# Daaohame/RAHT-3DGS-codec

Measured on AMD Instinct MI355X. Metric: M-Gaussians/s fwd+inv RAHT, 59-ch SH3 3DGS, higher is better.
Workload: dtype f32 (xyz columns: f64); 1 GPU; cfg3: 2999072 Gaussians (3000000 draws/GPU, J=12, 59 channels), fwd RAHT + quantize/reorder + dequantize/un-reorder + inv RAHT (quantization fused into the transform kernels); the 3 xyz columns carried in float64 inside the same launches (raht_fwd_quant_mixed / raht_dequant_inv_mixed): the reference's integers on every column; rows_per_gpu=2999072, channels=59, depth_J=12, engine=tile, quantize=True, parallelism=1 GPU, world=1

## Files before the change

### raht-3dgs-codec_amd/csrc/schedule.hip

```cpp
#include "raht_common.h"

#include <algorithm>
#include <atomic>

namespace raht {

__global__ void compact_scatter_kernel(const uint32_t *in, const uint32_t *flag, const uint32_t *pos, uint32_t *out, int64_t n);

__global__ void stage_survivor_kernel(const uint32_t *__restrict__ rows, int64_t n, int R, int64_t N,
                                      const int32_t *__restrict__ wl, const int32_t *__restrict__ wr,
                                      const uint8_t *__restrict__ lvl, int top_level,
                                      uint32_t *__restrict__ survivor)
{
    const int64_t j = (int64_t)blockIdx.x * blockDim.x + threadIdx.x;
    if (j >= n) return;
    const int64_t r = rows ? rows[j] : j;
    const int64_t t = j / R;
    const int64_t j0 = t * R, j1 = j0 + R;
    const int64_t start = rows ? rows[j0] : j0;
    const int64_t end = (j1 < n) ? (rows ? (int64_t)rows[j1] : j1) : N;
    const bool merged = (r > 0) && ((int)lvl[r] < top_level) && (r - wl[r] >= start) && (r + wr[r] <= end);
    survivor[j] = merged ? 0u : 1u;
}

// ... 378 lines not shown
        P.prog = st.prog;
        const size_t lds = st.rows ? (size_t)R * 4 : 0;
        const unsigned grid = (unsigned)st.n_tiles;
        by_lane_slots(R, [&](auto spl) {
            hipLaunchKernelGGL(tile_program_kernel<decltype(spl)::value>, dim3(grid), dim3(64), lds, s, P, plan->N, plan->top_level, plan->wsum);
        });
        RAHT_HIP_CHECK(hipGetLastError());
        st.prog_stride = P.stride; st.prog_ab = P.ab; st.prog_compact = P.compact != 0;
        built = true;
    }
    if (built) {
        if (!sc->ready) RAHT_HIP_CHECK(hipEventCreateWithFlags(&sc->ready.ev, hipEventDisableTiming));
        RAHT_HIP_CHECK(hipEventRecord(sc->ready, s));
        sc->ready_on = s;
    }
    return RAHT_OK;
}

__global__ void top_resolve_kernel(const uint32_t *__restrict__ rows, int64_t n, const int32_t *__restrict__ wl,
                                   const int32_t *__restrict__ wr, const uint8_t *__restrict__ lvl,
                                   const int64_t *__restrict__ wsum, int top_level, uint32_t *__restrict__ pj,
                                   double *__restrict__ ab, uint8_t *__restrict__ bucket, uint32_t *__restrict__ is_root)
{
    const int64_t e = (int64_t)blockIdx.x * blockDim.x + threadIdx.x;
    if (e >= n) return;
    const int64_t r = rows ? (int64_t)rows[e] : e;
    const int l = (int)lvl[r];
    const bool merged = (r > 0) && (l < top_level);
    is_root[e] = merged ? 0u : 1u;
    bucket[e] = merged ? (uint8_t)l : (uint8_t)63;
    uint32_t rec = 0;
    double a = 0.0, b = 0.0;
    if (merged) {
        const int64_t want = r - wl[r];
        int64_t p = want;
        if (rows) {
            int64_t lo = 0, hi = e - 1;
            while (lo < hi) {
                const int64_t mid = (lo + hi) >> 1;
                if ((int64_t)rows[mid] < want) lo = mid + 1; else hi = mid;
            }
            p = lo;
        }
        double w0, w1;
        pair_weights(r, wl[r], wr[r], wsum, w0, w1);
        const double den = w0 + w1;
        a = sqrt(w0 / den);
        b = sqrt(w1 / den);
        rec = (uint32_t)p | ((uint32_t)e << 16);
    }
    pj[e] = rec; ab[2 * e] = a; ab[2 * e + 1] = b;
}

__global__ void top_gather_kernel(const uint32_t *__restrict__ perm, uint32_t n_merges, const uint32_t *__restrict__ pj,
                                  const double *__restrict__ ab, uint32_t *__restrict__ t_pj,
                                  float *__restrict__ t_ab32, double *__restrict__ t_ab64)
{
    const uint32_t k = blockIdx.x * blockDim.x + threadIdx.x;
    if (k >= n_merges) return;
    const uint32_t e = perm[k];
    t_pj[k] = pj[e];
    const double a = ab[2 * e], b = ab[2 * e + 1];
    t_ab64[2 * k] = a; t_ab64[2 * k + 1] = b;
    t_ab32[2 * k] = (float)a; t_ab32[2 * k + 1] = (float)b;
}

__global__ void top_root_rank_kernel(const uint32_t *__restrict__ is_root, const uint32_t *__restrict__ pos, int64_t n,
                                     uint32_t *__restrict__ t_root)
{
    const int64_t e = (int64_t)blockIdx.x * blockDim.x + threadIdx.x;
    if (e < n) t_root[e] = is_root[e] ? pos[e] : 0xffffffffu;
}

static hipError_t gather_stage_meta(const raht_plan *plan, Stage &st, hipStream_t s)
{
    const size_t n = (size_t)st.n_entries;
    hipError_t e = hipSuccess;
    if ((e = st.e_wl.alloc(n)) != hipSuccess || (e = st.e_wr.alloc(n)) != hipSuccess || (e = st.e_lvl.alloc(n)) != hipSuccess ||
        (e = st.e_pos.alloc(n)) != hipSuccess) return e;
    hipLaunchKernelGGL(gather_meta_kernel, dim3((unsigned)ceil_div((int64_t)n, 256)), dim3(256), 0, s, st.rows, (int64_t)n, plan->wl,
                       plan->wr, plan->lvl, plan->inv_order, st.e_wl, st.e_wr, st.e_lvl, st.e_pos);
    return hipSuccess;
}

static int build_top_stage(raht_plan *plan, int64_t n, hipStream_t s, Stage &st)
{
    st.is_top = true;
    st.n_entries = n;
    st.n_tiles = 1;
    st.tile_rows = (int)n;
    const uint32_t *rows = st.rows;
    const unsigned gb = (unsigned)ceil_div(n, 256);
    if (rows) RAHT_HIP_CHECK(gather_stage_meta(plan, st, s));
    Scratch buf(sizeof(double) * 2 * (size_t)n + sizeof(uint32_t) * (4 * (size_t)n + 66) + (size_t)n, s);
    if (!buf.ok()) return RAHT_ERR_NOMEM;
    double *ab = buf.as<double>();
    uint32_t *pj = (uint32_t *)(ab + 2 * n), *is_root = pj + n, *pos = is_root + n, *perm = pos + n, *boff = perm + n,
             *total = boff + 65;
    uint8_t *bucket = (uint8_t *)(total + 1);
    hipLaunchKernelGGL(top_resolve_kernel, dim3(gb), dim3(256), 0, s, rows, n, plan->wl, plan->wr, plan->lvl, plan->wsum,
                       plan->top_level, pj, ab, bucket, is_root);
    RAHT_RET(exclusive_scan_u32(is_root, pos, n, total, s));
    RAHT_HIP_CHECK(st.t_root.alloc((size_t)n));
    hipLaunchKernelGGL(top_root_rank_kernel, dim3(gb), dim3(256), 0, s, is_root, pos, n, st.t_root);
    RAHT_RET(bucket_sort_u8(bucket, perm, n, 6, boff, s));
    RAHT_RET(read_back_u32(st.t_loff, boff, 65, nullptr, nullptr, 0, s));
    st.n_merges = st.t_loff[63];
    {
        uint32_t *lev = st.t_lev_host;
        int nlev = 0;
        for (int l = 0; l < 63; ++l)
            if (st.t_loff[l + 1] > st.t_loff[l]) { lev[2 * nlev] = st.t_loff[l]; lev[2 * nlev + 1] = st.t_loff[l + 1]; ++nlev; }
        int nbig = nlev;
        while (nbig > 0 && lev[2 * (nbig - 1) + 1] - lev[2 * (nbig - 1)] <= 64) --nbig;
        const size_t lds_budget = 160 * 1024 - 1024;
        while (nbig < nlev && (size_t)n * 16 + (size_t)(st.n_merges - lev[2 * nbig]) * 20 > lds_budget) ++nbig;
        st.t_nlev = nlev; st.t_nbig = nbig;
        st.t_small_start = (nbig < nlev) ? lev[2 * nbig] : st.n_merges;
        RAHT_HIP_CHECK(st.t_lev.alloc(2 * 64));
        RAHT_HIP_CHECK(hipMemcpyAsync(st.t_lev, lev, sizeof(uint32_t) * 2 * (size_t)std::max(nlev, 1), hipMemcpyHostToDevice, s));
    }
    const size_t nm = std::max<size_t>(st.n_merges, 1);
    RAHT_HIP_CHECK(st.t_pj.alloc(nm));
    RAHT_HIP_CHECK(st.t_ab32.alloc(2 * nm));
    RAHT_HIP_CHECK(st.t_ab64.alloc(2 * nm));
    if (st.n_merges)
        hipLaunchKernelGGL(top_gather_kernel, dim3((unsigned)ceil_div(st.n_merges, 256)), dim3(256), 0, s, perm, st.n_merges,
                           pj, ab, st.t_pj, st.t_ab32, st.t_ab64);
    return RAHT_OK;
}

constexpr int SB_THREADS = 256, SB_ITEMS = 8, SB_BLOCK = SB_THREADS * SB_ITEMS;
constexpr int SCHED_SPEC_MAX = 8;
enum { SK_NONE = 0, SK_TILE = 1, SK_TOP = 2 };

struct SchedState {
    uint32_t n[SCHED_SPEC_MAX + 2];
    uint32_t kind[SCHED_SPEC_MAX + 2];
    uint32_t finished;
    uint32_t last_stage, last_is_top;
    uint32_t trouble;
    uint32_t top[4];
};
constexpr int SCHED_STATE_WORDS = sizeof(SchedState) / 4;

__device__ __forceinline__ uint32_t block_sum_256(uint32_t v, uint32_t *red )
{
#pragma unroll
    for (int d = 32; d >= 1; d >>= 1) v += __shfl_xor(v, d, 64);
    if ((threadIdx.x & 63) == 0) red[threadIdx.x >> 6] = v;
    __syncthreads();
    const uint32_t t = red[0] + red[1] + red[2] + red[3];
    __syncthreads();
    return t;
}

__device__ __forceinline__ void sched_state_init(SchedState *S, uint32_t n0, uint32_t kind0)
// ... 104 lines not shown
#pragma unroll
        for (int q = 0; q < SB_ITEMS; ++q) { f[q] = (base + q < n) ? flags[base + q] : 0; mine += f[q]; }
    }
    uint32_t inc = mine;
    const int lane = threadIdx.x & 63, wid = threadIdx.x >> 6;
#pragma unroll
    for (int d = 1; d < 64; d <<= 1) { const uint32_t t = __shfl_up(inc, d, 64); if (lane >= d) inc += t; }
    if (lane == 63) wsum[wid] = inc;
    __syncthreads();
    uint32_t before = 0, block_tot = 0;
#pragma unroll
    for (int w = 0; w < 4; ++w) { if (w < wid) before += wsum[w]; block_tot += wsum[w]; }
    uint32_t pos = block_base + before + inc - mine;
    uint32_t tile = (uint32_t)base / (uint32_t)R;
    uint32_t next_start = tile * (uint32_t)R;
    if (next_start < (uint32_t)base) { ++tile; next_start += (uint32_t)R; }
    uint32_t g_r[SB_ITEMS], g_pos[SB_ITEMS], g_inv[SB_ITEMS];
    int32_t g_wl[SB_ITEMS], g_wr[SB_ITEMS];
    uint8_t g_lv[SB_ITEMS];
    bool keep[SB_ITEMS];
#pragma unroll
    for (int q = 0; q < SB_ITEMS; ++q) {
        const int64_t j = base + q;
        keep[q] = false; g_pos[q] = 0; g_r[q] = (uint32_t)j;
        if (j < n) {
            if ((uint32_t)j == next_start) { surv_off[tile] = pos; ++tile; next_start += (uint32_t)R; }
            if (f[q]) {
                keep[q] = pos < cap_next;
                g_pos[q] = pos;
                if (keep[q] && rows) g_r[q] = rows[j];
                ++pos;
            }
        }
    }
#pragma unroll
    for (int q = 0; q < SB_ITEMS; ++q) {
        g_wl[q] = 0; g_wr[q] = 0; g_lv[q] = 0; g_inv[q] = 0;
        if (keep[q]) { const uint32_t r = g_r[q]; g_wl[q] = p_wl[r]; g_wr[q] = p_wr[r]; g_lv[q] = p_lvl[r]; g_inv[q] = p_inv[r]; }
    }
#pragma unroll
    for (int q = 0; q < SB_ITEMS; ++q)
        if (keep[q]) { const uint32_t o = g_pos[q]; n_rows[o] = g_r[q]; n_wl[o] = g_wl[q]; n_wr[o] = g_wr[q]; n_lvl[o] = g_lv[q]; n_pos[o] = g_inv[q]; }
    if ((int64_t)blockIdx.x == nblk - 1 && threadIdx.x == 0) {
        const uint32_t total = block_base + block_tot;
        surv_off[(n + R - 1) / R] = total;
        S->n[k + 1] = total;
        if (total > cap_next) S->trouble = 1;
        else if (total == n_roots) { S->finished = 1; S->last_stage = (uint32_t)k; S->last_is_top = 0; }
        else if (total >= (uint32_t)n) S->trouble = 2;
        else S->kind[k + 1] = (total <= Rf) ? SK_TOP : SK_TILE;
    }
}

constexpr int ST_THREADS = 1024;
struct SchedTopOut { uint32_t *t_pj; float *t_ab32; double *t_ab64; uint32_t *t_root; uint32_t *t_lev; };

__device__ __forceinline__ void sched_top_body(SchedState *__restrict__ S, int k, int n, const uint32_t *__restrict__ rows,
                                               const int32_t *__restrict__ p_wl, const int32_t *__restrict__ p_wr,
                                               const uint8_t *__restrict__ p_lvl, const int64_t *__restrict__ wsum,
                                               int top_level, const SchedTopOut &O)
{
    __shared__ uint32_t s_rows[RAHT_TOP_MAX_ROWS];
    __shared__ uint32_t hist[64], cursor[64], wtot[ST_THREADS / 64];
    __shared__ uint32_t root_base;
    uint32_t *__restrict__ t_pj = O.t_pj, *__restrict__ t_root = O.t_root, *__restrict__ t_lev = O.t_lev;
    float *__restrict__ t_ab32 = O.t_ab32;
    double *__restrict__ t_ab64 = O.t_ab64;
    const int tid = threadIdx.x, lane = tid & 63, wid = tid >> 6;
    if (tid < 64) hist[tid] = 0;
    if (tid == 0) root_base = 0;
    for (int e = tid; e < n; e += ST_THREADS) s_rows[e] = rows ? rows[e] : (uint32_t)e;
    __syncthreads();
    PL_STAMP(2, 0, 8);
    for (int e0 = 0; e0 < n; e0 += ST_THREADS) {
        const int e = e0 + tid;
        bool root = false;
        if (e < n) {
            const uint32_t r = s_rows[e];
            const int l = (int)p_lvl[r];
            const bool merged = (r > 0) && (l < top_level);
            root = !merged;
            if (merged) atomicAdd(&hist[l], 1u);
        }
        const uint64_t bal = __ballot(root);
        if (lane == 0) wtot[wid] = (uint32_t)__popcll(bal);
        __syncthreads();
        uint32_t before = root_base;
        for (int w = 0; w < wid; ++w) before += wtot[w];
        if (e < n) t_root[e] = root ? before + (uint32_t)__popcll(bal & (((uint64_t)1 << lane) - 1)) : 0xffffffffu;
        __syncthreads();
        if (tid == 0) { uint32_t t = 0; for (int w = 0; w < ST_THREADS / 64; ++w) t += wtot[w]; root_base += t; }
        __syncthreads();
    }
    PL_STAMP(2, 0, 9);
    if (wid == 0) {
        const uint32_t h = (lane < 63) ? hist[lane] : 0u;
        uint32_t inc = h;
#pragma unroll
        for (int d = 1; d < 64; d <<= 1) { const uint32_t t = __shfl_up(inc, d, 64); if (lane >= d) inc += t; }
        const uint32_t first = inc - h;
        cursor[lane] = first;
        const uint32_t n_merges = (uint32_t)__shfl((int)inc, 63, 64);
        const uint64_t nonempty = __ballot(h > 0), below = ((uint64_t)1 << lane) - 1;
        const int nlev = __popcll(nonempty);
        const int my = __popcll(nonempty & below);
        if (h > 0) { t_lev[2 * my] = first; t_lev[2 * my + 1] = first + h; }
        const uint64_t big = __ballot(h > 64);
        int nbig = big ? __popcll(nonempty & (((uint64_t)2 << (63 - __clzll((long long)big))) - 1)) : 0;
        const size_t lds_budget = 160 * 1024 - 1024;
        uint32_t small_start = n_merges;
        for (;;) {
            uint32_t cand = n_merges;
            if (nbig < nlev) {
                const uint64_t owner = __ballot(h > 0 && my == nbig);
                cand = (uint32_t)__shfl((int)first, __ffsll((unsigned long long)owner) - 1, 64);
            }
            if (nbig < nlev && (size_t)n * 16 + (size_t)(n_merges - cand) * 20 > lds_budget) { ++nbig; continue; }
            small_start = cand;
            break;
        }
        if (lane == 0) {
            S->top[0] = n_merges; S->top[1] = (uint32_t)nlev; S->top[2] = (uint32_t)nbig; S->top[3] = small_start;
            S->finished = 1; S->last_stage = (uint32_t)k; S->last_is_top = 1;
        }
    }
    __syncthreads();
    PL_STAMP(2, 0, 10);
    for (int e = tid; e < n; e += ST_THREADS) {
        const uint32_t r = s_rows[e];
        const int l = (int)p_lvl[r];
        if (!((r > 0) && (l < top_level))) continue;
        const int32_t wlr = p_wl[r], wrr = p_wr[r];
        const uint32_t want = r - (uint32_t)wlr;
        int lo = 0, hi = e - 1;
        while (lo < hi) {
            const int mid = (lo + hi) >> 1;
            if (s_rows[mid] < want) lo = mid + 1; else hi = mid;
        }
        double w0, w1;
        pair_weights((int64_t)r, wlr, wrr, wsum, w0, w1);
        const double den = w0 + w1;
        const double a = sqrt(w0 / den), b = sqrt(w1 / den);
        const uint32_t pos = atomicAdd(&cursor[l], 1u);
        t_pj[pos] = (uint32_t)lo | ((uint32_t)e << 16);
        t_ab64[2 * pos] = a; t_ab64[2 * pos + 1] = b;
        t_ab32[2 * pos] = (float)a; t_ab32[2 * pos + 1] = (float)b;
    }
    PL_STAMP(2, 0, 11);
}

struct SchedStageBufs {
    uint32_t *rows[SCHED_SPEC_MAX + 2]; int32_t *wl[SCHED_SPEC_MAX + 2], *wr[SCHED_SPEC_MAX + 2];
    uint8_t *lvl[SCHED_SPEC_MAX + 2]; uint32_t *pos[SCHED_SPEC_MAX + 2], *surv[SCHED_SPEC_MAX + 2];
    uint32_t cap[SCHED_SPEC_MAX + 2];
};

__global__ __launch_bounds__(ST_THREADS) void sched_tail_kernel(SchedState *S, int k_multi, int k_last, SchedStageBufs B, int R, uint32_t Rf,
                                                                uint32_t n_roots, int64_t N, int top_level, uint32_t tail_max,
                                                                const int32_t *__restrict__ p_wl, const int32_t *__restrict__ p_wr,
                                                                const uint8_t *__restrict__ p_lvl, const uint32_t *__restrict__ p_inv,
                                                                const int64_t *__restrict__ wsum, SchedTopOut O, int64_t n_first)
{
    __shared__ uint32_t wcnt[8 * (ST_THREADS / 64)], woff[8 * (ST_THREADS / 64) + 1];
    __shared__ uint32_t s_kind[SCHED_SPEC_MAX + 2], s_n[SCHED_SPEC_MAX + 2];
    const int tid = threadIdx.x, lane = tid & 63, wid = tid >> 6;
    PL_SLOT_DECL;
    PL_STAMP_NEXT();
    if (n_first >= 0) { sched_state_init(S, (uint32_t)n_first, SK_TOP); __builtin_amdgcn_fence(__ATOMIC_RELEASE, "workgroup"); __syncthreads(); }
    if (tid < SCHED_SPEC_MAX + 2) {
        s_kind[tid] = (n_first >= 0) ? (tid == 0 ? (uint32_t)SK_TOP : (uint32_t)SK_NONE) : __atomic_load_n(&S->kind[tid], __ATOMIC_RELAXED);
        s_n[tid] = (n_first >= 0) ? (tid == 0 ? (uint32_t)n_first : 0u) : __atomic_load_n(&S->n[tid], __ATOMIC_RELAXED);
    }
    __syncthreads();
    for (int k = (k_multi == 0) ? 0 : 1; k <= k_last; ++k) {
        const uint32_t kind = s_kind[k], n = s_n[k];
        PL_STAMP_NEXT();
        if (kind == SK_TOP) {
            sched_top_body(S, k, (int)n, B.rows[k], p_wl, p_wr, p_lvl, wsum, top_level, O);
            return;
        }
        if (kind == SK_TILE && k < k_multi) continue;
        if (kind != SK_TILE || n > tail_max || n > B.cap[k] || k == k_last) return;
        const uint32_t *__restrict__ rows = B.rows[k];
        const int32_t *__restrict__ wl = B.wl[k], *__restrict__ wr = B.wr[k];
        const uint8_t *__restrict__ lvl = B.lvl[k];
        uint32_t *__restrict__ surv_off = B.surv[k];
        uint32_t *__restrict__ n_rows = B.rows[k + 1], *__restrict__ n_pos = B.pos[k + 1];
        int32_t *__restrict__ n_wl = B.wl[k + 1], *__restrict__ n_wr = B.wr[k + 1];
        uint8_t *__restrict__ n_lvl = B.lvl[k + 1];
        const uint32_t cap_next = B.cap[k + 1];
        uint32_t running = 0;
        constexpr int TI = 8, NWV = ST_THREADS / 64;
        for (uint32_t base = 0; base < n; base += ST_THREADS * TI) {
            uint32_t r[TI], e_start[TI], e_end[TI];
            int32_t e_wl[TI], e_wr[TI];
            uint8_t e_lv[TI];
            uint64_t bal[TI];
// ... 293 lines not shown
```

### raht-3dgs-codec_amd/csrc/transform.hip

```cpp
#include "raht_common.h"
#include "raht_device.h"
#include "tile_engine.h"
#include "tile_host.h"

#include <algorithm>
#include <type_traits>
#include <vector>

namespace raht {

size_t tile_lds_bytes(int R, int elem_size, int Dc, bool ident, bool qm);

template <typename T> struct Vec16;
template <> struct Vec16<float> { typedef float4 type; static constexpr int n = 4; };
template <> struct Vec16<double> { typedef double2 type; static constexpr int n = 2; };

template <typename T>
__global__ void copy_rows_kernel(const T *__restrict__ src, int64_t lds, T *__restrict__ dst, int64_t ldd,
                                 int64_t N, int D)
{
    const int64_t total = N * D;
    for (int64_t e = (int64_t)blockIdx.x * blockDim.x + threadIdx.x; e < total;
         e += (int64_t)gridDim.x * blockDim.x) {
        const int64_t i = e / D;
// ... 635 lines not shown
template <typename T>
struct TileBatch {
    TileArgs<T> a[BATCH_MAX];
    uint32_t first_tile[BATCH_MAX + 1];
    int n;
};

template <typename T, bool INV, bool IDENT, bool QM, int SLOTS>
__global__ __launch_bounds__(TILE_THREADS, (sizeof(T) == 4 ? 6 : 4)) void tile_kernel_batch(const TileBatch<T> B,
                                                   const typename std::conditional<QM, typename StepsFor<T>::type, NoSteps>::type ST)
{
    int s = 0;
#pragma unroll
    for (int q = 1; q < BATCH_MAX; ++q) s += (q < B.n && blockIdx.x >= B.first_tile[q]) ? 1 : 0;
    const int64_t t = (int64_t)(blockIdx.x - B.first_tile[s]);
    tile_body<T, INV, IDENT, QM, SLOTS>(B.a[s], ST, t, (int64_t)1 << 40, (int)blockIdx.y);
}

constexpr int TOP_THREADS = 1024;
constexpr int TOP_SLOTS = RAHT_TOP_MAX_ROWS / TOP_THREADS;

template <typename T>
struct TopArgs {
    const T *in;  int64_t ld_in;
    T *fin;       int64_t ld_fin;
    T *out;       int64_t ld_out;
    int32_t *Q;   int64_t ldq;
    const uint32_t *rows;
    int io_mapped;
    const uint32_t *e_pos;
    const uint32_t *pj;
    const T *ab;
    const uint32_t *root_rank;
    T *root_buf;
    int n, n_merges, D;
    const uint32_t *lev;
    int nlev, nbig;
    uint32_t small_start;
};

template <typename T, bool INV, bool QM, bool MULTI = false>
__device__ __forceinline__ void top_body(const TopArgs<T> &A, const typename std::conditional<QM, typename StepsFor<T>::type, NoSteps>::type &ST,
                                         const int chunk, const MultiQ *MQ = nullptr)
{
    constexpr bool QM64 = QM && sizeof(T) == 8;
    extern __shared__ __align__(16) unsigned char smem[];
    typedef RegChunk<T> V16;
    constexpr int VN = 16 / sizeof(T);
    V16 *tile = (V16 *)smem;
    __shared__ uint32_t s_lev[2 * 64];
    const int tid = threadIdx.x;
    const int goff = min(chunk * VN, A.D - VN);
    const int n = A.n, nm = A.n_merges;
    if (tid < 2 * A.nlev) s_lev[tid] = A.lev[tid];
    const int n_small = nm - (int)A.small_start;
    uint32_t *s_pj = (uint32_t *)(smem + (size_t)n * 16);
    T *s_ab = (T *)(s_pj + ((n_small + 3) & ~3));
    for (int i = tid; i < n_small; i += TOP_THREADS) {
        s_pj[i] = A.pj[A.small_start + i];
        s_ab[2 * i] = A.ab[2 * (A.small_start + i)];
        s_ab[2 * i + 1] = A.ab[2 * (A.small_start + i) + 1];
    }

    typename StepsFor<T>::elem my_step[VN];
    float my_rcp[VN];
#pragma unroll
    for (int i = 0; i < VN; ++i) { my_step[i] = 1; my_rcp[i] = 1.0f; }
    if constexpr (QM) {
#pragma unroll
        for (int i = 0; i < VN; ++i) {
            my_step[i] = ST.v[ST.n == 1 ? 0 : goff + i];
            if constexpr (!QM64) my_rcp[i] = refined_rcp(my_step[i]);
        }
    }

    uint32_t pj[TOP_SLOTS];
    T ra[TOP_SLOTS], rb[TOP_SLOTS];
#pragma unroll
    for (int k = 0; k < TOP_SLOTS; ++k) {
        const int idx = min(k * TOP_THREADS + tid, max(nm - 1, 0));
        pj[k] = A.pj[idx]; ra[k] = A.ab[2 * idx]; rb[k] = A.ab[2 * idx + 1];
    }
    uint32_t m_dst[TOP_SLOTS], m_rr[TOP_SLOTS];
#pragma unroll
    for (int k = 0; k < TOP_SLOTS; ++k) {
        const int e = min(k * TOP_THREADS + tid, n - 1);
        m_rr[k] = A.root_rank[e];
        m_dst[k] = QM ? A.e_pos[e] : (A.rows ? A.rows[e] : (uint32_t)e);
    }
    {
        typedef typename std::conditional<QM && INV && !QM64, int32_t, T>::type RawT;
        RegChunk<RawT> x[TOP_SLOTS];
#pragma unroll
        for (int k = 0; k < TOP_SLOTS; ++k) {
            const int e = min(k * TOP_THREADS + tid, n - 1);
            if constexpr (QM64 && INV) {
                int32_t q[VN];
                ld_ints<VN>(A.Q + (int64_t)m_dst[k] * A.ldq + goff, q);
#pragma unroll
                for (int i = 0; i < VN; ++i) x[k].v[i] = (T)q[i];
            } else if constexpr (!INV) {
                x[k] = ld_chunk<RawT>((const RawT *)A.in + (int64_t)(A.io_mapped ? m_dst[k] : (uint32_t)e) * A.ld_in + goff);
            } else if constexpr (QM) {
                x[k] = ld_chunk<RawT>((const RawT *)A.Q + (int64_t)m_dst[k] * A.ldq + goff);
            } else {
                const T *src = (A.root_buf && m_rr[k] != 0xffffffffu) ? A.root_buf + (int64_t)m_rr[k] * A.D
                                                                      : A.fin + (int64_t)m_dst[k] * A.ld_fin;
                x[k] = ld_chunk<RawT>((const RawT *)src + goff);
            }
        }
#pragma unroll
        for (int k = 0; k < TOP_SLOTS; ++k) {
            const int e = k * TOP_THREADS + tid;
            if (e < n) {
                V16 v;
#pragma unroll
                for (int i = 0; i < VN; ++i) {
                    v.v[i] = (T)x[k].v[i];
                    if constexpr (QM && INV) v.v[i] = v.v[i] * (T)my_step[i];
                }
                tile[e] = v;
            }
        }
        if constexpr (QM && INV) {
            if (A.root_buf) {
#pragma unroll
                for (int k = 0; k < TOP_SLOTS; ++k) {
                    const int e = k * TOP_THREADS + tid;
                    if (e < n && m_rr[k] != 0xffffffffu) tile[e] = ld_chunk<T>(A.root_buf + (int64_t)m_rr[k] * A.D + goff);
                }
            }
        }
    }
    __syncthreads();

    auto butterfly = [&](uint32_t rec, T a, T b) {
        const uint32_t ip = rec & 0xffffu, ij = rec >> 16;
        const V16 x0 = tile[ip], x1 = tile[ij];
        V16 vlo, vhi;
#pragma unroll
        for (int i = 0; i < VN; ++i) {
            if (!INV) {
                vlo.v[i] = a * x0.v[i] + b * x1.v[i];
                vhi.v[i] = a * x1.v[i] - b * x0.v[i];
            } else {
                vlo.v[i] = a * x0.v[i] - b * x1.v[i];
                vhi.v[i] = b * x0.v[i] + a * x1.v[i];
            }
        }
        tile[ip] = vlo; tile[ij] = vhi;
    };
    auto big_levels = [&]() {
#pragma unroll 1
        for (int q = 0; q < A.nbig; ++q) {
            const int li = INV ? A.nbig - 1 - q : q;
            const uint32_t lo = s_lev[2 * li], hi = s_lev[2 * li + 1];
#pragma unroll
            for (int k = 0; k < TOP_SLOTS; ++k) {
                const uint32_t idx = (uint32_t)(k * TOP_THREADS + tid);
                if ((uint32_t)(k * TOP_THREADS) < hi && (uint32_t)((k + 1) * TOP_THREADS) > lo && idx >= lo && idx < hi)
                    butterfly(pj[k], ra[k], rb[k]);
            }
            __syncthreads();
        }
    };
    auto small_levels = [&]() {
        if (tid < 64) {
#pragma unroll 1
            for (int q = A.nbig; q < A.nlev; ++q) {
                const int li = INV ? A.nlev - 1 - (q - A.nbig) : q;
                const uint32_t lo = s_lev[2 * li], hi = s_lev[2 * li + 1];
                const uint32_t i = lo - A.small_start + (uint32_t)tid;
                if (lo + (uint32_t)tid < hi) butterfly(s_pj[i], s_ab[2 * i], s_ab[2 * i + 1]);
            }
        }
        __syncthreads();
    };
    if (!INV) { big_levels(); small_levels(); }
    else { small_levels(); big_levels(); }

#pragma unroll
    for (int k = 0; k < TOP_SLOTS; ++k) {
        const int e = k * TOP_THREADS + tid;
        if (e >= n) continue;
        const V16 v = tile[e];
        if constexpr (INV) {
            st_chunk<T>(A.out + (int64_t)(A.io_mapped ? m_dst[k] : (uint32_t)e) * A.ld_out + goff, v);
        } else {
            const uint32_t rr = m_rr[k];
            const bool to_buf = A.root_buf && rr != 0xffffffffu;
            if (to_buf) st_chunk<T>(A.root_buf + (int64_t)rr * A.D + goff, v);
            if (QM && to_buf) {
            } else if constexpr (QM) {
                if constexpr (QM64) {
                    int32_t qv[VN];
#pragma unroll
                    for (int i = 0; i < VN; ++i) qv[i] = quantize_one_f64((double)v.v[i], (double)my_step[i]);
                    st_ints<VN>(A.Q + (int64_t)m_dst[k] * A.ldq + goff, qv);
                } else if constexpr (MULTI) {
                    for (int kk = 0; kk < MQ->k; ++kk) {
                        const float sp = MQ->step[kk], rc = refined_rcp(sp);
                        RegChunk<int32_t> qv;
#pragma unroll
                        for (int i = 0; i < VN; ++i) qv.v[i] = quantize_one((float)v.v[i], sp, rc, MQ->fast_div);
                        st_chunk<int32_t>(MQ->Q[kk] + (int64_t)m_dst[k] * A.ldq + goff, qv);
                    }
                } else {
                    RegChunk<int32_t> qv;
#pragma unroll
                    for (int i = 0; i < VN; ++i) qv.v[i] = quantize_one((float)v.v[i], (float)my_step[i], my_rcp[i], ST.fast_div);
                    st_chunk<int32_t>(A.Q + (int64_t)m_dst[k] * A.ldq + goff, qv);
                }
            } else {
                st_chunk<T>(A.fin + (int64_t)m_dst[k] * A.ld_fin + goff, v);
            }
        }
    }
}

template <typename T, bool INV, bool QM>
__global__ __launch_bounds__(TOP_THREADS) void top_kernel(const TopArgs<T> A,
                                                          const typename std::conditional<QM, typename StepsFor<T>::type, NoSteps>::type ST)
{
    top_body<T, INV, QM>(A, ST, (int)blockIdx.x);
}

// ... 707 lines not shown
```

### raht-3dgs-codec_amd/csrc/transform_mx.hip

```cpp
#include "raht_common.h"
#include "raht_device.h"
#include "tile_engine.h"
#include "tile_host.h"

#include <algorithm>
#include <cstdlib>
#include <string>
#include <type_traits>
#include <vector>

namespace raht {

#ifdef RAHT_PHASE_CLOCKS
constexpr int MX_CLK_TILES = 4096, MX_CLK_SLOTS = 12;
__device__ unsigned long long g_phase_clk_mx[MX_CLK_TILES][MX_CLK_SLOTS];
#define MX_STAMP(k) do { if (IDENT && threadIdx.x == 0 && tile_id < MX_CLK_TILES) g_phase_clk_mx[tile_id][k] = __builtin_readcyclecounter(); } while (0)
#else
#define MX_STAMP(k) do { } while (0)
#endif

constexpr int MX_MAX_WIDE = 4;
constexpr int MX_THREADS = 512;
constexpr int MX_TOP_THREADS = 1024;
constexpr int MX_TOP_SLOTS = RAHT_TOP_MAX_ROWS / MX_TOP_THREADS;
// ... 580 lines not shown
__global__ __launch_bounds__(MX_THREADS, 6) void tile_kernel_mx_sq(const TileArgs<float> A, const MxPtrs P, const StepTableMX ST)
{
    tile_body_mx<true, true, SLOTS, false, false, true>(A, P, ST, (int64_t)blockIdx.x);
}

struct TileBatchMX {
    TileArgs<float> a[BATCH_MAX];
    MxPtrs p[BATCH_MAX];
    uint32_t first_tile[BATCH_MAX + 1];
    int n;
};
static_assert(sizeof(TileBatchMX) + sizeof(StepTableMX) <= 4096, "tile_kernel_mx_batch: arguments exceed the 4 KB kernarg segment");

template <bool INV, bool IDENT, int SLOTS>
__global__ __launch_bounds__(MX_THREADS, 6) void tile_kernel_mx_batch(const TileBatchMX B, const StepTableMX ST)
{
    int s = 0;
#pragma unroll
    for (int q = 1; q < BATCH_MAX; ++q) s += (q < B.n && blockIdx.x >= B.first_tile[q]) ? 1 : 0;
    tile_body_mx<INV, IDENT, SLOTS, false>(B.a[s], B.p[s], ST, (int64_t)(blockIdx.x - B.first_tile[s]));
}

struct TopArgsMX {
    const float *in_rows;  int64_t ld_in;
    const float *in_img; const double *in_img_w;
    float *out_rows;       int64_t ld_out;
    float *out_img; double *out_img_w;
    int32_t *Q;            int64_t ldq;
    const uint32_t *e_pos;
    const uint32_t *pj;
    const float *ab32;  const double *ab64;
    int n, n_merges, D, nwide, Fp;
    const uint32_t *lev;
    int nlev, nbig;
    uint32_t small_start;
    const uint32_t *root_rank;
    float *root_f; double *root_w;
};

template <bool WIDE, bool INV, bool ROOTS, bool MULTI = false>
__device__ __forceinline__ void top_body_mx(const TopArgsMX &A, const StepTableMX &ST, const int chunk, const MxMultiQ *MQ = nullptr)
{
    typedef typename std::conditional<WIDE, double, float>::type T;
    constexpr int VN = WIDE ? 2 : 4;
    typedef RegChunk<T> V16;
    extern __shared__ __align__(16) unsigned char smem[];
    V16 *tile = (V16 *)smem;
    __shared__ uint32_t s_lev[2 * 64];
    const int tid = threadIdx.x;
    const int nwide = A.nwide;
    const int goff = WIDE ? 2 * chunk : min(chunk * 4, A.D - 4);
    const int ioff = chunk * 4;
    const int n = A.n, nm = A.n_merges;
    if (tid < 2 * A.nlev) s_lev[tid] = A.lev[tid];
    const T *ab = WIDE ? (const T *)A.ab64 : (const T *)A.ab32;
    const int n_small = nm - (int)A.small_start;
    uint32_t *s_pj = (uint32_t *)(smem + (size_t)n * 16);
    T *s_ab = (T *)(s_pj + ((n_small + 3) & ~3));
    for (int i = tid; i < n_small; i += MX_TOP_THREADS) {
        s_pj[i] = A.pj[A.small_start + i];
        s_ab[2 * i] = ab[2 * (A.small_start + i)];
        s_ab[2 * i + 1] = ab[2 * (A.small_start + i) + 1];
    }
    T my_step[VN];
    float my_rcp[VN];
    bool live[VN];
#pragma unroll
    for (int i = 0; i < VN; ++i) {
        if constexpr (WIDE) { live[i] = goff + i < nwide; my_step[i] = live[i] ? ST.w[goff + i] : 1.0; my_rcp[i] = 1.0f; }
        else { live[i] = !(chunk == 0 && i < nwide); my_step[i] = ST.f.v[ST.f.n == 1 ? 0 : goff + i]; my_rcp[i] = refined_rcp(my_step[i]); }
    }
    uint32_t pj[MX_TOP_SLOTS];
    T ra[MX_TOP_SLOTS], rb[MX_TOP_SLOTS];
#pragma unroll
    for (int k = 0; k < MX_TOP_SLOTS; ++k) {
        const int idx = min(k * MX_TOP_THREADS + tid, max(nm - 1, 0));
        pj[k] = A.pj[idx]; ra[k] = ab[2 * idx]; rb[k] = ab[2 * idx + 1];
    }
    uint32_t m_dst[MX_TOP_SLOTS], m_rr[MX_TOP_SLOTS];
#pragma unroll
    for (int k = 0; k < MX_TOP_SLOTS; ++k) {
        m_dst[k] = A.e_pos[min(k * MX_TOP_THREADS + tid, n - 1)];
        m_rr[k] = ROOTS ? A.root_rank[min(k * MX_TOP_THREADS + tid, n - 1)] : 0xffffffffu;
    }
#pragma unroll
    for (int k = 0; k < MX_TOP_SLOTS; ++k) {
        const int e = k * MX_TOP_THREADS + tid;
        if (e >= n) continue;
        V16 v;
        if constexpr (!INV) {
            if (A.in_img) {
                if constexpr (WIDE) {
#pragma unroll
                    for (int i = 0; i < VN; ++i) v.v[i] = live[i] ? A.in_img_w[(int64_t)e * nwide + goff + i] : 0.0;
                } else {
                    v = *(const V16 *)(A.in_img + (int64_t)e * A.Fp + ioff);
                }
            } else if constexpr (WIDE) {
#pragma unroll
                for (int i = 0; i < VN; ++i) v.v[i] = live[i] ? (double)A.in_rows[(int64_t)e * A.ld_in + goff + i] : 0.0;
            } else {
                v = ld_chunk<float>(A.in_rows + (int64_t)e * A.ld_in + goff);
            }
        } else if (m_rr[k] != 0xffffffffu) {
            if constexpr (WIDE) {
#pragma unroll
                for (int i = 0; i < VN; ++i) v.v[i] = live[i] ? A.root_w[(int64_t)m_rr[k] * nwide + goff + i] : 0.0;
            } else {
                v = ld_chunk<float>(A.root_f + (int64_t)m_rr[k] * A.D + goff);
            }
        } else {
            const int32_t *q = A.Q + (int64_t)m_dst[k] * A.ldq + goff;
            if constexpr (WIDE) {
#pragma unroll
                for (int i = 0; i < VN; ++i) v.v[i] = live[i] ? (double)q[i] * my_step[i] : 0.0;
            } else {
                const RegChunk<int32_t> raw = ld_chunk<int32_t>(q);
#pragma unroll
                for (int i = 0; i < VN; ++i) v.v[i] = (float)raw.v[i] * my_step[i];
            }
        }
        tile[e] = v;
    }
    __syncthreads();

    auto butterfly = [&](uint32_t rec, T a, T b) {
        const uint32_t ip = rec & 0xffffu, ij = rec >> 16;
        const V16 x0 = tile[ip], x1 = tile[ij];
        V16 vlo, vhi;
#pragma unroll
        for (int i = 0; i < VN; ++i) {
            if (!INV) {
                vlo.v[i] = a * x0.v[i] + b * x1.v[i];
                vhi.v[i] = a * x1.v[i] - b * x0.v[i];
            } else {
                vlo.v[i] = a * x0.v[i] - b * x1.v[i];
                vhi.v[i] = b * x0.v[i] + a * x1.v[i];
            }
        }
        tile[ip] = vlo; tile[ij] = vhi;
    };
    auto big_levels = [&]() {
#pragma unroll 1
        for (int q = 0; q < A.nbig; ++q) {
            const int li = INV ? A.nbig - 1 - q : q;
            const uint32_t lo = s_lev[2 * li], hi = s_lev[2 * li + 1];
#pragma unroll
            for (int k = 0; k < MX_TOP_SLOTS; ++k) {
                const uint32_t idx = (uint32_t)(k * MX_TOP_THREADS + tid);
                if ((uint32_t)(k * MX_TOP_THREADS) < hi && (uint32_t)((k + 1) * MX_TOP_THREADS) > lo && idx >= lo && idx < hi)
                    butterfly(pj[k], ra[k], rb[k]);
            }
            __syncthreads();
        }
    };
    auto small_levels = [&]() {
        if (tid < 64) {
#pragma unroll 1
            for (int q = A.nbig; q < A.nlev; ++q) {
                const int li = INV ? A.nlev - 1 - (q - A.nbig) : q;
                const uint32_t lo = s_lev[2 * li], hi = s_lev[2 * li + 1];
                const uint32_t i = lo - A.small_start + (uint32_t)tid;
                if (lo + (uint32_t)tid < hi) butterfly(s_pj[i], s_ab[2 * i], s_ab[2 * i + 1]);
            }
        }
        __syncthreads();
    };
    if (!INV) { big_levels(); small_levels(); }
    else { small_levels(); big_levels(); }

#pragma unroll
    for (int k = 0; k < MX_TOP_SLOTS; ++k) {
        const int e = k * MX_TOP_THREADS + tid;
        if (e >= n) continue;
        const V16 v = tile[e];
        if constexpr (INV) {
            if (A.out_img) {
                if constexpr (WIDE) {
#pragma unroll
                    for (int i = 0; i < VN; ++i) if (live[i]) A.out_img_w[(int64_t)e * nwide + goff + i] = v.v[i];
                } else {
                    *(V16 *)(A.out_img + (int64_t)e * A.Fp + ioff) = v;
                }
            } else if constexpr (WIDE) {
#pragma unroll
                for (int i = 0; i < VN; ++i) if (live[i]) A.out_rows[(int64_t)e * A.ld_out + goff + i] = (float)v.v[i];
            } else if (chunk == 0) {
#pragma unroll
                for (int i = 0; i < VN; ++i) if (live[i]) A.out_rows[(int64_t)e * A.ld_out + goff + i] = v.v[i];
            } else {
                st_chunk<float>(A.out_rows + (int64_t)e * A.ld_out + goff, v);
            }
        } else if (m_rr[k] != 0xffffffffu) {
            if constexpr (WIDE) {
#pragma unroll
                for (int i = 0; i < VN; ++i) if (live[i]) A.root_w[(int64_t)m_rr[k] * nwide + goff + i] = v.v[i];
            } else {
                st_chunk<float>(A.root_f + (int64_t)m_rr[k] * A.D + goff, v);
            }
        } else if constexpr (MULTI) {
            for (int kk = 0; kk < MQ->k; ++kk) {
                int32_t *q = MQ->Q[kk] + (int64_t)m_dst[k] * A.ldq + goff;
                if constexpr (WIDE) {
#pragma unroll
                    for (int i = 0; i < VN; ++i) if (live[i]) q[i] = quantize_one_f64(v.v[i], MQ->step[kk]);
                } else {
                    const float sf = (float)MQ->step[kk], rf = refined_rcp(sf);
                    const int fd = (int)((MQ->fast_div >> kk) & 1u);
                    RegChunk<int32_t> qv;
#pragma unroll
                    for (int i = 0; i < VN; ++i) qv.v[i] = quantize_one(v.v[i], sf, rf, fd);
                    if (chunk == 0) {
#pragma unroll
                        for (int i = 0; i < VN; ++i) if (live[i]) q[i] = qv.v[i];
                    } else {
                        st_chunk<int32_t>(q, qv);
// ... 702 lines not shown
```

Baseline: 4902 M-Gaussians/s.

## Regroup top-stage merges by subtree height and prefetch small-level butterflies

The top-stage schedule now buckets merges by their dependency height in the merge tree rather than by octree level. This should produce fewer, fuller levels, so the top kernel needs fewer barriers and serial small-level steps. The top transform kernels issue their global input loads before staging the small-level table into LDS from registers. The small-level loop is software-pipelined, using readlane-broadcast level bounds and double-buffered record fetches to hide LDS latency. The risks are extra scheduling work (a height pass with a barrier per level and a binary search moved earlier) and higher register pressure from holding all input chunks at once.

Measured after the change: 4897 M-Gaussians/s. No clear change (-0.1%).

```diff
diff --git a/raht-3dgs-codec_amd/csrc/schedule.hip b/raht-3dgs-codec_amd/csrc/schedule.hip
--- a/raht-3dgs-codec_amd/csrc/schedule.hip
+++ b/raht-3dgs-codec_amd/csrc/schedule.hip
@@ -454,6 +454,61 @@
     pj[e] = rec; ab[2 * e] = a; ab[2 * e + 1] = b;
 }
 
+constexpr int HT_TOP_THREADS = 1024, HT_TOP_SLOTS = RAHT_TOP_MAX_ROWS / HT_TOP_THREADS;
+static_assert(HT_TOP_SLOTS == 8 && RAHT_TOP_MAX_ROWS <= 1 << 16, "top_heights: a byte per slot in 64 bits, 16-bit entry indices");
+constexpr uint64_t HT_TOP_NONE = 0x3f3f3f3f3f3f3f3full;
+__device__ __forceinline__ uint64_t top_heights(int n, const uint32_t *present, const uint16_t *s_part, uint8_t *s_h, uint64_t lv8)
+{
+    const int tid = threadIdx.x;
+    for (int e = tid; e < n; e += HT_TOP_THREADS) s_h[e] = 0;
+    uint64_t ht8 = 0;
+    __syncthreads();
+#pragma unroll 1
+    for (uint32_t l = 0; l < 63; ++l) {
+        if (present[l] == 0) continue;
+#pragma unroll
+        for (int k = 0; k < HT_TOP_SLOTS; ++k) {
+            if ((uint32_t)(lv8 >> (8 * k) & 0xffu) != l) continue;
+            const int e = k * HT_TOP_THREADS + tid;
+            const uint32_t ip = s_part[e];
+            const uint32_t h0 = s_h[ip], h1 = s_h[e];
+            const uint32_t h = 1 + (h0 > h1 ? h0 : h1);
+            s_h[ip] = (uint8_t)h;
+            ht8 |= (uint64_t)h << (8 * k);
+        }
+        __syncthreads();
+    }
+    return ht8;
+}
+
+__global__ __launch_bounds__(HT_TOP_THREADS) void top_heights_kernel(int n, const uint32_t *__restrict__ pj, uint8_t *__restrict__ bucket)
+{
+    __shared__ uint8_t s_h[RAHT_TOP_MAX_ROWS];
+    __shared__ uint16_t s_part[RAHT_TOP_MAX_ROWS];
+    __shared__ uint32_t present[64];
+    const int tid = threadIdx.x;
+    if (tid < 64) present[tid] = 0;
+    __syncthreads();
+    uint64_t lv8 = HT_TOP_NONE;
+#pragma unroll
+    for (int k = 0; k < HT_TOP_SLOTS; ++k) {
+        const int e = k * HT_TOP_THREADS + tid;
+        if (e >= n) continue;
+        const uint32_t l = bucket[e];
+        s_part[e] = (uint16_t)(pj[e] & 0xffffu);
+        lv8 = (lv8 & ~((uint64_t)0xff << (8 * k))) | ((uint64_t)l << (8 * k));
+        if (l != 63) present[l] = 1;
+    }
+    __syncthreads();
+    const uint64_t ht8 = top_heights(n, present, s_part, s_h, lv8);
+#pragma unroll
+    for (int k = 0; k < HT_TOP_SLOTS; ++k) {
+        const int e = k * HT_TOP_THREADS + tid;
+        const uint32_t h = (uint32_t)(ht8 >> (8 * k)) & 0xffu;
+        if (e < n && h != 0) bucket[e] = (uint8_t)(h - 1);
+    }
+}
+
 __global__ void top_gather_kernel(const uint32_t *__restrict__ perm, uint32_t n_merges, const uint32_t *__restrict__ pj,
                                   const double *__restrict__ ab, uint32_t *__restrict__ t_pj,
                                   float *__restrict__ t_ab32, double *__restrict__ t_ab64)
@@ -505,6 +560,7 @@
     RAHT_RET(exclusive_scan_u32(is_root, pos, n, total, s));
     RAHT_HIP_CHECK(st.t_root.alloc((size_t)n));
     hipLaunchKernelGGL(top_root_rank_kernel, dim3(gb), dim3(256), 0, s, is_root, pos, n, st.t_root);
+    hipLaunchKernelGGL(top_heights_kernel, dim3(1), dim3(HT_TOP_THREADS), 0, s, (int)n, pj, bucket);
     RAHT_RET(bucket_sort_u8(bucket, perm, n, 6, boff, s));
     RAHT_RET(read_back_u32(st.t_loff, boff, 65, nullptr, nullptr, 0, s));
     st.n_merges = st.t_loff[63];
@@ -715,7 +771,7 @@
     }
 }
 
-constexpr int ST_THREADS = 1024;
+constexpr int ST_THREADS = HT_TOP_THREADS;
 struct SchedTopOut { uint32_t *t_pj; float *t_ab32; double *t_ab64; uint32_t *t_root; uint32_t *t_lev; };
 
 __device__ __forceinline__ void sched_top_body(SchedState *__restrict__ S, int k, int n, const uint32_t *__restrict__ rows,
@@ -724,13 +780,15 @@
                                                int top_level, const SchedTopOut &O)
 {
     __shared__ uint32_t s_rows[RAHT_TOP_MAX_ROWS];
-    __shared__ uint32_t hist[64], cursor[64], wtot[ST_THREADS / 64];
+    __shared__ uint8_t s_h[RAHT_TOP_MAX_ROWS];
+    __shared__ uint16_t s_part[RAHT_TOP_MAX_ROWS];
+    __shared__ uint32_t lhist[64], hist[64], cursor[64], wtot[ST_THREADS / 64];
     __shared__ uint32_t root_base;
     uint32_t *__restrict__ t_pj = O.t_pj, *__restrict__ t_root = O.t_root, *__restrict__ t_lev = O.t_lev;
     float *__restrict__ t_ab32 = O.t_ab32;
     double *__restrict__ t_ab64 = O.t_ab64;
     const int tid = threadIdx.x, lane = tid & 63, wid = tid >> 6;
-    if (tid < 64) hist[tid] = 0;
+    if (tid < 64) { lhist[tid] = 0; hist[tid] = 0; }
     if (tid == 0) root_base = 0;
     for (int e = tid; e < n; e += ST_THREADS) s_rows[e] = rows ? rows[e] : (uint32_t)e;
     __syncthreads();
@@ -743,7 +801,7 @@
             const int l = (int)p_lvl[r];
             const bool merged = (r > 0) && (l < top_level);
             root = !merged;
-            if (merged) atomicAdd(&hist[l], 1u);
+            if (merged) atomicAdd(&lhist[l], 1u);
         }
         const uint64_t bal = __ballot(root);
         if (lane == 0) wtot[wid] = (uint32_t)__popcll(bal);
@@ -755,6 +813,30 @@
         if (tid == 0) { uint32_t t = 0; for (int w = 0; w < ST_THREADS / 64; ++w) t += wtot[w]; root_base += t; }
         __syncthreads();
     }
+    uint64_t lv8 = HT_TOP_NONE;
+#pragma unroll 1
+    for (int q = 0; q * ST_THREADS < n; ++q) {
+        const int e = q * ST_THREADS + tid;
+        if (e >= n) continue;
+        const uint32_t r = s_rows[e];
+        const int l = (int)p_lvl[r];
+        if (!((r > 0) && (l < top_level))) continue;
+        const uint32_t want = r - (uint32_t)p_wl[r];
+        int lo = 0, hi = e - 1;
+        while (lo < hi) {
+            const int mid = (lo + hi) >> 1;
+            if (s_rows[mid] < want) lo = mid + 1; else hi = mid;
+        }
+        s_part[e] = (uint16_t)lo;
+        lv8 = (lv8 & ~((uint64_t)0xff << (8 * q))) | ((uint64_t)l << (8 * q));
+    }
+    const uint64_t ht8 = top_heights(n, lhist, s_part, s_h, lv8);
+#pragma unroll 1
+    for (int q = 0; q * ST_THREADS < n; ++q) {
+        const uint32_t h = (uint32_t)(ht8 >> (8 * q)) & 0xffu;
+        if (h != 0) atomicAdd(&hist[h - 1], 1u);
+    }
+    __syncthreads();
     PL_STAMP(2, 0, 9);
     if (wid == 0) {
         const uint32_t h = (lane < 63) ? hist[lane] : 0u;
@@ -789,23 +871,19 @@
     }
     __syncthreads();
     PL_STAMP(2, 0, 10);
-    for (int e = tid; e < n; e += ST_THREADS) {
-        const uint32_t r = s_rows[e];
-        const int l = (int)p_lvl[r];
-        if (!((r > 0) && (l < top_level))) continue;
+#pragma unroll 1
+    for (int q = 0; q * ST_THREADS < n; ++q) {
+        const uint32_t h = (uint32_t)(ht8 >> (8 * q)) & 0xffu;
+        if (h == 0) continue;
+        const int e = q * ST_THREADS + tid;
+        const uint32_t r = s_rows[e], lo = s_part[e];
         const int32_t wlr = p_wl[r], wrr = p_wr[r];
-        const uint32_t want = r - (uint32_t)wlr;
-        int lo = 0, hi = e - 1;
-        while (lo < hi) {
-            const int mid = (lo + hi) >> 1;
-            if (s_rows[mid] < want) lo = mid + 1; else hi = mid;
-        }
         double w0, w1;
         pair_weights((int64_t)r, wlr, wrr, wsum, w0, w1);
         const double den = w0 + w1;
         const double a = sqrt(w0 / den), b = sqrt(w1 / den);
-        const uint32_t pos = atomicAdd(&cursor[l], 1u);
-        t_pj[pos] = (uint32_t)lo | ((uint32_t)e << 16);
+        const uint32_t pos = atomicAdd(&cursor[h - 1], 1u);
+        t_pj[pos] = lo | ((uint32_t)e << 16);
         t_ab64[2 * pos] = a; t_ab64[2 * pos + 1] = b;
         t_ab32[2 * pos] = (float)a; t_ab32[2 * pos + 1] = (float)b;
     }
diff --git a/raht-3dgs-codec_amd/csrc/transform.hip b/raht-3dgs-codec_amd/csrc/transform.hip
--- a/raht-3dgs-codec_amd/csrc/transform.hip
+++ b/raht-3dgs-codec_amd/csrc/transform.hip
@@ -711,15 +711,10 @@
     const int tid = threadIdx.x;
     const int goff = min(chunk * VN, A.D - VN);
     const int n = A.n, nm = A.n_merges;
-    if (tid < 2 * A.nlev) s_lev[tid] = A.lev[tid];
+    const uint32_t lev_w = (tid < 2 * A.nlev) ? A.lev[tid] : 0u;
     const int n_small = nm - (int)A.small_start;
     uint32_t *s_pj = (uint32_t *)(smem + (size_t)n * 16);
     T *s_ab = (T *)(s_pj + ((n_small + 3) & ~3));
-    for (int i = tid; i < n_small; i += TOP_THREADS) {
-        s_pj[i] = A.pj[A.small_start + i];
-        s_ab[2 * i] = A.ab[2 * (A.small_start + i)];
-        s_ab[2 * i + 1] = A.ab[2 * (A.small_start + i) + 1];
-    }
 
     typename StepsFor<T>::elem my_step[VN];
     float my_rcp[VN];
@@ -749,6 +744,17 @@
     }
     {
         typedef typename std::conditional<QM && INV && !QM64, int32_t, T>::type RawT;
+        auto stage_table = [&]() {
+            if (tid < 2 * A.nlev) s_lev[tid] = lev_w;
+#pragma unroll
+            for (int k = 0; k < TOP_SLOTS; ++k) {
+                const int idx = k * TOP_THREADS + tid;
+                if (idx >= (int)A.small_start && idx < nm) {
+                    const int i = idx - (int)A.small_start;
+                    s_pj[i] = pj[k]; s_ab[2 * i] = ra[k]; s_ab[2 * i + 1] = rb[k];
+                }
+            }
+        };
         RegChunk<RawT> x[TOP_SLOTS];
 #pragma unroll
         for (int k = 0; k < TOP_SLOTS; ++k) {
@@ -768,6 +774,7 @@
                 x[k] = ld_chunk<RawT>((const RawT *)src + goff);
             }
         }
+        stage_table();
 #pragma unroll
         for (int k = 0; k < TOP_SLOTS; ++k) {
             const int e = k * TOP_THREADS + tid;
@@ -825,12 +832,28 @@
     };
     auto small_levels = [&]() {
         if (tid < 64) {
+            const int nsm = A.nlev - A.nbig;
+            const int mine = A.nbig + min(tid, max(nsm - 1, 0));
+            const int r_lo = (int)s_lev[2 * mine], r_hi = (int)s_lev[2 * mine + 1];
+            auto fetch = [&](int q, uint32_t &rec, T &a, T &b, bool &on) {
+                const int j = INV ? nsm - 1 - q : q;
+                const uint32_t lo = (uint32_t)__builtin_amdgcn_readlane(r_lo, j), hi = (uint32_t)__builtin_amdgcn_readlane(r_hi, j);
+                on = lo + (uint32_t)tid < hi;
+                const uint32_t i = on ? lo - A.small_start + (uint32_t)tid : 0u;
+                rec = s_pj[i]; a = s_ab[2 * i]; b = s_ab[2 * i + 1];
+            };
+            uint32_t rec0 = 0, rec1 = 0;
+            T a0 = 0, b0 = 0, a1 = 0, b1 = 0;
+            bool on0 = false, on1 = false;
+            if (nsm > 0) fetch(0, rec0, a0, b0, on0);
 #pragma unroll 1
-            for (int q = A.nbig; q < A.nlev; ++q) {
-                const int li = INV ? A.nlev - 1 - (q - A.nbig) : q;
-                const uint32_t lo = s_lev[2 * li], hi = s_lev[2 * li + 1];
-                const uint32_t i = lo - A.small_start + (uint32_t)tid;
-                if (lo + (uint32_t)tid < hi) butterfly(s_pj[i], s_ab[2 * i], s_ab[2 * i + 1]);
+            for (int q = 0; q < nsm; q += 2) {
+                on1 = false;
+                if (q + 1 < nsm) fetch(q + 1, rec1, a1, b1, on1);
+                if (on0) butterfly(rec0, a0, b0);
+                on0 = false;
+                if (q + 2 < nsm) fetch(q + 2, rec0, a0, b0, on0);
+                if (on1) butterfly(rec1, a1, b1);
             }
         }
         __syncthreads();
diff --git a/raht-3dgs-codec_amd/csrc/transform_mx.hip b/raht-3dgs-codec_amd/csrc/transform_mx.hip
--- a/raht-3dgs-codec_amd/csrc/transform_mx.hip
+++ b/raht-3dgs-codec_amd/csrc/transform_mx.hip
@@ -656,24 +656,21 @@
     const int goff = WIDE ? 2 * chunk : min(chunk * 4, A.D - 4);
     const int ioff = chunk * 4;
     const int n = A.n, nm = A.n_merges;
-    if (tid < 2 * A.nlev) s_lev[tid] = A.lev[tid];
     const T *ab = WIDE ? (const T *)A.ab64 : (const T *)A.ab32;
     const int n_small = nm - (int)A.small_start;
     uint32_t *s_pj = (uint32_t *)(smem + (size_t)n * 16);
     T *s_ab = (T *)(s_pj + ((n_small + 3) & ~3));
-    for (int i = tid; i < n_small; i += MX_TOP_THREADS) {
-        s_pj[i] = A.pj[A.small_start + i];
-        s_ab[2 * i] = ab[2 * (A.small_start + i)];
-        s_ab[2 * i + 1] = ab[2 * (A.small_start + i) + 1];
-    }
     T my_step[VN];
     float my_rcp[VN];
     bool live[VN];
+    int lch[VN];
 #pragma unroll
     for (int i = 0; i < VN; ++i) {
         if constexpr (WIDE) { live[i] = goff + i < nwide; my_step[i] = live[i] ? ST.w[goff + i] : 1.0; my_rcp[i] = 1.0f; }
         else { live[i] = !(chunk == 0 && i < nwide); my_step[i] = ST.f.v[ST.f.n == 1 ? 0 : goff + i]; my_rcp[i] = refined_rcp(my_step[i]); }
-    }
+        lch[i] = goff + (live[i] ? i : 0);
+    }
+    const uint32_t lev_w = (tid < 2 * A.nlev) ? A.lev[tid] : 0u;
     uint32_t pj[MX_TOP_SLOTS];
     T ra[MX_TOP_SLOTS], rb[MX_TOP_SLOTS];
 #pragma unroll
@@ -687,42 +684,75 @@
         m_dst[k] = A.e_pos[min(k * MX_TOP_THREADS + tid, n - 1)];
         m_rr[k] = ROOTS ? A.root_rank[min(k * MX_TOP_THREADS + tid, n - 1)] : 0xffffffffu;
     }
+    V16 x[MX_TOP_SLOTS];
+    if constexpr (!INV) {
+        if (A.in_img) {
+#pragma unroll
+            for (int k = 0; k < MX_TOP_SLOTS; ++k) {
+                const int64_t e = min(k * MX_TOP_THREADS + tid, n - 1);
+                if constexpr (WIDE) {
+#pragma unroll
+                    for (int i = 0; i < VN; ++i) x[k].v[i] = A.in_img_w[e * nwide + lch[i]];
+                } else {
+                    x[k] = *(const V16 *)(A.in_img + e * A.Fp + ioff);
+                }
+            }
+        } else {
+#pragma unroll
+            for (int k = 0; k < MX_TOP_SLOTS; ++k) {
+                const int64_t e = min(k * MX_TOP_THREADS + tid, n - 1);
+                if constexpr (WIDE) {
+#pragma unroll
+                    for (int i = 0; i < VN; ++i) x[k].v[i] = (double)A.in_rows[e * A.ld_in + lch[i]];
+                } else {
+                    x[k] = ld_chunk<float>(A.in_rows + e * A.ld_in + goff);
+                }
+            }
+        }
+    }
+    if (tid < 2 * A.nlev) s_lev[tid] = lev_w;
+#pragma unroll
+    for (int k = 0; k < MX_TOP_SLOTS; ++k) {
+        const int idx = k * MX_TOP_THREADS + tid;
+        if (idx >= (int)A.small_start && idx < nm) {
+            const int i = idx - (int)A.small_start;
+            s_pj[i] = pj[k]; s_ab[2 * i] = ra[k]; s_ab[2 * i + 1] = rb[k];
+        }
+    }
+    if constexpr (INV) {
+#pragma unroll
+        for (int k = 0; k < MX_TOP_SLOTS; ++k) {
+            const int32_t *q = A.Q + (int64_t)m_dst[k] * A.ldq;
+            if constexpr (WIDE) {
+#pragma unroll
+                for (int i = 0; i < VN; ++i) x[k].v[i] = (double)q[lch[i]] * my_step[i];
+            } else {
+                const RegChunk<int32_t> raw = ld_chunk<int32_t>(q + goff);
+#pragma unroll
+                for (int i = 0; i < VN; ++i) x[k].v[i] = (float)raw.v[i] * my_step[i];
+            }
+        }
+        if constexpr (ROOTS) {
+#pragma unroll
+            for (int k = 0; k < MX_TOP_SLOTS; ++k) {
+                if (m_rr[k] == 0xffffffffu) continue;
+                if constexpr (WIDE) {
+#pragma unroll
+                    for (int i = 0; i < VN; ++i) x[k].v[i] = A.root_w[(int64_t)m_rr[k] * nwide + lch[i]];
+                } else {
+                    x[k] = ld_chunk<float>(A.root_f + (int64_t)m_rr[k] * A.D + goff);
+                }
+            }
+        }
+    }
 #pragma unroll
     for (int k = 0; k < MX_TOP_SLOTS; ++k) {
         const int e = k * MX_TOP_THREADS + tid;
         if (e >= n) continue;
-        V16 v;
-        if constexpr (!INV) {
-            if (A.in_img) {
-                if constexpr (WIDE) {
-#pragma unroll
-                    for (int i = 0; i < VN; ++i) v.v[i] = live[i] ? A.in_img_w[(int64_t)e * nwide + goff + i] : 0.0;
-                } else {
-                    v = *(const V16 *)(A.in_img + (int64_t)e * A.Fp + ioff);
-                }
-            } else if constexpr (WIDE) {
-#pragma unroll
-                for (int i = 0; i < VN; ++i) v.v[i] = live[i] ? (double)A.in_rows[(int64_t)e * A.ld_in + goff + i] : 0.0;
-            } else {
-                v = ld_chunk<float>(A.in_rows + (int64_t)e * A.ld_in + goff);
-            }
-        } else if (m_rr[k] != 0xffffffffu) {
-            if constexpr (WIDE) {
-#pragma unroll
-                for (int i = 0; i < VN; ++i) v.v[i] = live[i] ? A.root_w[(int64_t)m_rr[k] * nwide + goff + i] : 0.0;
-            } else {
-                v = ld_chunk<float>(A.root_f + (int64_t)m_rr[k] * A.D + goff);
-            }
-        } else {
-            const int32_t *q = A.Q + (int64_t)m_dst[k] * A.ldq + goff;
-            if constexpr (WIDE) {
-#pragma unroll
-                for (int i = 0; i < VN; ++i) v.v[i] = live[i] ? (double)q[i] * my_step[i] : 0.0;
-            } else {
-                const RegChunk<int32_t> raw = ld_chunk<int32_t>(q);
-#pragma unroll
-                for (int i = 0; i < VN; ++i) v.v[i] = (float)raw.v[i] * my_step[i];
-            }
+        V16 v = x[k];
+        if constexpr (WIDE) {
+#pragma unroll
+            for (int i = 0; i < VN; ++i) if (!live[i]) v.v[i] = 0.0;
         }
         tile[e] = v;
     }
@@ -760,12 +790,28 @@
     };
     auto small_levels = [&]() {
         if (tid < 64) {
+            const int nsm = A.nlev - A.nbig;
+            const int mine = A.nbig + min(tid, max(nsm - 1, 0));
+            const int r_lo = (int)s_lev[2 * mine], r_hi = (int)s_lev[2 * mine + 1];
+            auto fetch = [&](int q, uint32_t &rec, T &a, T &b, bool &on) {
+                const int j = INV ? nsm - 1 - q : q;
+                const uint32_t lo = (uint32_t)__builtin_amdgcn_readlane(r_lo, j), hi = (uint32_t)__builtin_amdgcn_readlane(r_hi, j);
+                on = lo + (uint32_t)tid < hi;
+                const uint32_t i = on ? lo - A.small_start + (uint32_t)tid : 0u;
+                rec = s_pj[i]; a = s_ab[2 * i]; b = s_ab[2 * i + 1];
+            };
+            uint32_t rec0 = 0, rec1 = 0;
+            T a0 = 0, b0 = 0, a1 = 0, b1 = 0;
+            bool on0 = false, on1 = false;
+            if (nsm > 0) fetch(0, rec0, a0, b0, on0);
 #pragma unroll 1
-            for (int q = A.nbig; q < A.nlev; ++q) {
-                const int li = INV ? A.nlev - 1 - (q - A.nbig) : q;
-                const uint32_t lo = s_lev[2 * li], hi = s_lev[2 * li + 1];
-                const uint32_t i = lo - A.small_start + (uint32_t)tid;
-                if (lo + (uint32_t)tid < hi) butterfly(s_pj[i], s_ab[2 * i], s_ab[2 * i + 1]);
+            for (int q = 0; q < nsm; q += 2) {
+                on1 = false;
+                if (q + 1 < nsm) fetch(q + 1, rec1, a1, b1, on1);
+                if (on0) butterfly(rec0, a0, b0);
+                on0 = false;
+                if (q + 2 < nsm) fetch(q + 2, rec0, a0, b0, on0);
+                if (on1) butterfly(rec1, a1, b1);
             }
         }
         __syncthreads();
```
